# lschoenm/MerKurio

Hardware: AMD Instinct MI355X
Metric: Gbases/s scanned (150bp FASTQ, 10k 31-mers); % HBM roofline at 1/2/4/8 GPUs (higher is better)
Workload: dtype u8

## Files before the change

merkurio_amd/csrc/matcher.cpp:

```cpp
#include <hip/hip_runtime.h>

#include <algorithm>
#include <chrono>
#include <cmath>
#include <cstdarg>
#include <cstdio>
#include <cstdlib>
#include <cstring>
#include <memory>
#include <string>
#include <vector>

#include "host_common.h"
#include "matcher_internal.h"
#include "scan_kernel.h"

namespace mk {

thread_local char g_last_error[512] = "";

int fail(int code, const char *fmt, ...) {
    va_list ap;
    va_start(ap, fmt);
    vsnprintf(g_last_error, sizeof(g_last_error), fmt, ap);
// ... 519 lines not shown
    p.pat_bytes = m->d_pat_bytes;
    p.pat_off = m->d_pat_off;
    p.n_pat = m->n_pat;
    p.q = m->q;
    const uint64_t kmask = m->q >= 32 ? ~0ull : ((1ull << (2 * m->q)) - 1);
    p.key_mask_lo = (uint32_t)kmask;
    p.key_mask_hi = (uint32_t)(kmask >> 32);
    p.case_insensitive = (m->flags & MK_FLAG_ASCII_CASE_INSENSITIVE) ? 1 : 0;
    p.s2 = m->split_len ? m->S2 : 0;
    p.s2_log2 = m->S2 >= 8 ? 3 : m->S2 >= 4 ? 2 : m->S2 >= 2 ? 1 : 0;
    p.key2_mask = (1u << (2 * m->q2)) - 1u;
    p.short_bytes = m->q2 <= kShortByteMaxQ;
    p.short_bitmap = m->d_short_table;
    p.uniform_len = m->uniform_len;
    p.rec_flags32 = (uint32_t *)d_rec_flags;
    p.hits = (mk_hit *)d_hits;
    p.hits_cap = (mode == MK_MODE_HITS) ? hits_cap : 0;
    p.n_hits = (unsigned long long *)d_n_hits;
    p.counters = (unsigned long long *)d_counters;
    p.error_word = m->d_error;
    const uint64_t waves_per_block = kBlockThreads / 64;
    uint64_t blocks = (n_tiles + waves_per_block - 1) / waves_per_block;
    if (blocks > (uint64_t)m->num_cus) blocks = m->num_cus;
    p.stage = m->d_stage;
    p.rec_per_byte = (double)n_rec / (double)n_bytes;
    const uint64_t tiles_per_wave = n_tiles / (blocks * waves_per_block);
    p.tile_run = m->tile_run ? m->tile_run : tiles_per_wave >= 16 ? 4 : tiles_per_wave >= 8 ? 2 : 1;
    p.rec_index = nullptr;
    p.rec_len = rec_len;
    p.inv_rec_len = rec_len ? 1.0 / (double)rec_len : 0.0;
    if (m->ragged && !rec_len && n_rec < (1ull << 32)) {
        int rc_i = ensure((void **)&m->d_rec_index, &m->d_rec_index_cap, ((n_bytes >> kRecIndexShift) + 2) * sizeof(uint32_t));
        if (rc_i) return rc_i;
        launch_rec_index(p.rec_off, n_rec, n_bytes, m->d_rec_index, st);
        p.rec_index = m->d_rec_index;
    }
    const size_t slots = m->ev_start.size();
    const size_t slot = slots ? (size_t)(m->timed_launches % slots) : 0;
    if (slots) MK_HIP(hipEventRecord(m->ev_start[slot], st));
    const uint32_t kDensePerMille = mode == MK_MODE_HITS ? 95 : 145;
    const bool plain_loads = m->hit_density_pm >= kDensePerMille && !m->split_len;
    const int flavour = plain_loads ? 0 : 1;
    const bool listed = !(plain_loads && m->gbloom_blocks == 0) && mode != MK_MODE_HITS && n_rec < (1ull << 32);
    p.flag_list = listed ? m->d_flag_list : nullptr;
    p.flag_counts = m->d_flag_counts;
    p.flag_cap = kFlagListCap;
    const char *name = launch_scan(p, (int)m->S, m->q > 16, mode == MK_MODE_HITS, m->gbloom_blocks != 0, flavour, (int)blocks, st);
    if (!name) return fail(MK_E_UNSUPPORTED, "no kernel for stride %u", m->S);
    if (slots) {
        MK_HIP(hipEventRecord(m->ev_stop[slot], st));
        m->timed_launches++;
    }
    if (listed)
        launch_flag_scatter(m->d_flag_list, m->d_flag_counts, kFlagListCap, (uint32_t)(blocks * waves_per_block), (uint8_t *)d_rec_flags, st);
    if (d_counters) {
        launch_count_flags(p, st);
        if (mode == MK_MODE_HITS && p.hits && p.hits_cap) launch_hist_hits(p, m->num_cus, st);
    }
    m->kernel_name = name;
    m->last_grid = (int)blocks;
    MK_HIP(hipGetLastError());
    return MK_OK;
}

static int take_device_errors(mk_matcher *m, hipStream_t st) {
    uint32_t w = 0;
    MK_HIP(hipMemcpyAsync(&w, m->d_error, sizeof(w), hipMemcpyDeviceToHost, st));
    MK_HIP(hipStreamSynchronize(st));
    if (!w) return MK_OK;
    MK_HIP(hipMemsetAsync(m->d_error, 0, sizeof(w), st));
    return fail(MK_E_UNSUPPORTED, "an occurrence lies 4 GiB or more into its record: a single record must be shorter than 4 GiB "
                                  "(mk_hit.pos is 32 bits); the tuples of that scan are not usable");
}

int mk_matcher_check_device(mk_matcher *m, void *stream) {
    if (!m) return fail(MK_E_INVALID_ARG, "null matcher");
    MK_HIP(hipSetDevice(m->device));
    return take_device_errors(m, (hipStream_t)stream);
}

int mk_matcher_hint_hit_density(mk_matcher *m, uint32_t records_hit_per_1000) {
    if (!m) return fail(MK_E_INVALID_ARG, "null matcher");
    m->hit_density_pm = records_hit_per_1000 > 1000 ? 1000 : records_hit_per_1000;
    return MK_OK;
}

int mk_matcher_set_fixed_record_length(mk_matcher *m, uint32_t record_length) {
    if (!m) return fail(MK_E_INVALID_ARG, "null matcher");
    m->fixed_rec_len = record_length;
    return MK_OK;
}

int mk_matcher_hint_record_lengths(mk_matcher *m, int equal_lengths) {
    if (!m) return fail(MK_E_INVALID_ARG, "null matcher");
    m->ragged = !equal_lengths;
    return MK_OK;
}

int mk_matcher_enable_timing(mk_matcher *m, uint32_t slots) {
    if (!m) return fail(MK_E_INVALID_ARG, "null matcher");
    MK_ABI_BEGIN
    MK_HIP(hipSetDevice(m->device));
    for (auto e : m->ev_start) (void)hipEventDestroy(e);
    for (auto e : m->ev_stop) (void)hipEventDestroy(e);
    m->ev_start.assign(slots, nullptr);
    m->ev_stop.assign(slots, nullptr);
    m->timed_launches = 0;
    for (uint32_t i = 0; i < slots; ++i) {
        MK_HIP(hipEventCreate(&m->ev_start[i]));
// ... 353 lines not shown
```

merkurio_amd/csrc/scan_kernel.h:

```cpp
#pragma once
#include <hip/hip_runtime.h>
#include <stdint.h>

#include "../../include/merkurio_hip.h"
#include "filter.hpp"

namespace mk {

constexpr uint32_t kHitStage = 1024;
constexpr uint32_t kFlagListCap = 2048;

struct ScanParams {
    const uint8_t *seq;
    uint64_t n_bytes;
    const uint64_t *rec_off;
    uint64_t n_rec;
    const uint32_t *bloom;
    uint32_t gbloom_blocks;
    const TableEntry *table;
    uint32_t table_mask;
    const uint8_t *pat_bytes;
    const uint32_t *pat_off;
    uint32_t n_pat;
    uint32_t q;
    uint32_t key_mask_lo;
    uint32_t key_mask_hi;
    uint32_t s2;
    uint32_t s2_log2;
    uint32_t key2_mask;
    uint32_t short_bytes;
    const uint32_t *short_bitmap;
    uint32_t case_insensitive;
    uint32_t uniform_len;
    double rec_per_byte;
    uint32_t tile_run;
    const uint32_t *rec_index;
    uint32_t rec_len;
    double inv_rec_len;
    mk_hit *stage;
    uint32_t *rec_flags32;
    uint32_t *flag_list;
    uint32_t *flag_counts;
    uint32_t flag_cap;
    mk_hit *hits;
    uint64_t hits_cap;
    unsigned long long *n_hits;
    unsigned long long *counters;
    uint32_t *error_word;
};

const char *launch_scan(const ScanParams &p, int S, bool wide, bool emit, bool global_filter, int flavour, int grid_blocks,
                        hipStream_t stream);

template <int S, int QC, bool EMIT, bool GF, int FL, int MC = 0>
void launch_variant(const ScanParams &p, int grid_blocks, hipStream_t stream);

uint32_t scan_lds_bytes();

void launch_hist_hits(const ScanParams &p, int grid_blocks, hipStream_t stream);

constexpr uint32_t kRecIndexShift = 16;
void launch_clear(uint32_t *flags32, uint64_t n_words, unsigned long long *n_hits, hipStream_t stream);
void launch_flag_scatter(const uint32_t *flag_list, const uint32_t *flag_counts, uint32_t flag_cap, uint32_t n_waves, uint8_t *rec_flags,
                         hipStream_t stream);
void launch_rec_index(const uint64_t *rec_off, uint64_t n_rec, uint64_t n_bytes, uint32_t *rec_index, hipStream_t stream);
struct OrderKey {
    const uint32_t *pat_off;
    uint32_t uniform_len;
    const uint32_t *rank;
    const uint32_t *unrank;
    uint64_t rec_base;
    uint32_t ac;
    uint32_t bits_a;
    uint32_t bits_b;
    uint32_t b_hi;
    uint32_t b_lo;
    uint32_t shift;
    uint32_t n_bins;
};
struct OrderScratch {
    unsigned long long *stats;
    uint32_t *g_cnt;
    uint32_t *bin_start;
    uint32_t *cursor;
    uint32_t *big_list;
    uint64_t *keys;
};
constexpr uint32_t kOrderMaxBins = 32768;
constexpr uint32_t kOrderLeafMax = 16384;
constexpr uint32_t kOrderLeafSmall = 4096;
void launch_order_hist(const mk_hit *d_hits, uint64_t n, const OrderKey &L, const OrderScratch &S, int num_cus, hipStream_t st);
void launch_order_scatter_leaf(mk_hit *d_hits, uint64_t n, const OrderKey &L, const OrderScratch &S, uint32_t max_bin, uint32_t n_big,
                               int num_cus, hipStream_t st);
hipError_t order_kernels_prepare();
hipError_t order_hits_library(mk_hit *d_hits, size_t n, bool ac, const uint32_t *d_pat_off, uint32_t uniform_len, void *tmp,
                              size_t *tmp_bytes, hipStream_t stream);

void launch_pattern_sets(const mk_hit *d_hits, uint64_t n, uint64_t n_rec, uint32_t *d_found_pat, unsigned long long *d_found_off,
                         unsigned long long *d_total, void *d_tile, hipStream_t st);
void launch_count_u32(const uint32_t *d_list, uint64_t n, uint32_t *d_counts, uint32_t n_bins, hipStream_t st);
void launch_rows(const mk_hit *d_hits, uint64_t n, uint32_t file, mk_row *d_rows, hipStream_t st);
void launch_pair_mark(mk_hit *d_hits, uint64_t n, uint32_t mate, bool ac, hipStream_t st);
void launch_rows_pair(const mk_hit *d_hits, uint64_t n, bool ac, mk_row *d_rows, hipStream_t st);
void launch_count_pair_heads(const mk_hit *d_hits, uint64_t n, uint32_t *d_counts, uint32_t n_bins, hipStream_t st);

void launch_ingest_count(const uint8_t *d_text, uint64_t n, uint32_t *d_block_cnt, uint32_t *d_total, hipStream_t st);
void launch_ingest_records(const uint8_t *d_text, uint64_t n, const uint32_t *d_block_off, const uint32_t *d_total, uint32_t *d_line_start,
                           uint64_t n_rec, uint32_t *d_rec_start, uint32_t *d_seq_start, uint32_t *d_seq_len, uint32_t *d_status, hipStream_t st);
void launch_ingest_lines(const uint8_t *d_text, uint64_t n, const uint32_t *d_block_off, const uint32_t *d_total, uint32_t *d_line_start, hipStream_t st);
void launch_ingest_offsets(const uint32_t *d_seq_len, uint64_t n_rec, unsigned long long *d_tile, unsigned long long *d_off, hipStream_t st);
void launch_ingest_gather(const uint8_t *d_text, const uint32_t *d_seq_start, const uint32_t *d_seq_len, const unsigned long long *d_off,
                          uint32_t fixed_len, uint64_t n_rec, uint8_t *d_seq, hipStream_t st, uint32_t skip_from = 0xFFFFFFFFu);
void launch_ingest_select(const uint8_t *d_flags, uint32_t invert, const uint32_t *d_rec_start, uint64_t n_rec, uint32_t n_text, uint32_t *d_sel_len,
                          hipStream_t st);
void launch_ingest_fasta_count(const uint8_t *d_text, uint64_t n, const uint32_t *d_nl_block_off, const uint32_t *d_line_start,
                               unsigned long long *d_block64, hipStream_t st);
void launch_ingest_fasta_emit(const uint8_t *d_text, uint64_t n, const uint32_t *d_nl_block_off, const uint32_t *d_line_start,
// ... 71 lines not shown
```

merkurio_amd/csrc/scan_kernel.hip:

```cpp
#include <algorithm>

#include "scan_kernel.h"

namespace mk {

__global__ __launch_bounds__(1024) void mk_count_flags_kernel(const uint8_t *__restrict__ flags, uint64_t n_rec,
                                                             unsigned long long *__restrict__ out) {
    const uint64_t head = std::min<uint64_t>(n_rec, (16 - ((uintptr_t)flags & 15)) & 15);
    const uint64_t n16 = (n_rec - head) / 16;
    const uint4 *__restrict__ v = reinterpret_cast<const uint4 *>(flags + head);
    unsigned long long c = 0;
    const uint64_t stride = (uint64_t)gridDim.x * blockDim.x;
    uint64_t i = (uint64_t)blockIdx.x * blockDim.x + threadIdx.x;
    for (; i + 3 * stride < n16; i += 4 * stride) {
        const uint4 a = v[i], b = v[i + stride], d = v[i + 2 * stride], e = v[i + 3 * stride];
        c += __popc(a.x) + __popc(a.y) + __popc(a.z) + __popc(a.w) + __popc(b.x) + __popc(b.y) + __popc(b.z) + __popc(b.w) +
             __popc(d.x) + __popc(d.y) + __popc(d.z) + __popc(d.w) + __popc(e.x) + __popc(e.y) + __popc(e.z) + __popc(e.w);
    }
    for (; i < n16; i += stride) {
        const uint4 a = v[i];
        c += __popc(a.x) + __popc(a.y) + __popc(a.z) + __popc(a.w);
    }
    if (blockIdx.x == 0 && threadIdx.x == 0) {
        for (uint64_t r = 0; r < head; ++r) c += flags[r] != 0;
        for (uint64_t r = head + n16 * 16; r < n_rec; ++r) c += flags[r] != 0;
    }
    __shared__ unsigned long long part[16];
    for (int o = 32; o > 0; o >>= 1) c += __shfl_down(c, o);
    if ((threadIdx.x & 63) == 0) part[threadIdx.x >> 6] = c;
    __syncthreads();
    if (threadIdx.x == 0) {
        unsigned long long t = 0;
        for (unsigned w = 0; w < blockDim.x / 64; ++w) t += part[w];
        if (t) atomicAdd(out, t);
    }
}

void launch_count_flags(const ScanParams &p, hipStream_t st) {
    const uint64_t n16 = p.n_rec / 16;
    const int blocks = (int)std::min<uint64_t>(256, std::max<uint64_t>(1, (n16 + 4095) / 4096));
    hipLaunchKernelGGL(mk_count_flags_kernel, dim3(blocks), dim3(1024), 0, st, reinterpret_cast<const uint8_t *>(p.rec_flags32),
                       p.n_rec, p.counters + p.n_pat + MK_SUM_RECORDS_HIT);
}

__global__ __launch_bounds__(1024) void mk_clear_kernel(uint32_t *__restrict__ flags32, uint64_t n_words,
                                                       unsigned long long *__restrict__ n_hits) {
    if (blockIdx.x == 0 && threadIdx.x == 0) *n_hits = 0;
    const uint64_t head = std::min<uint64_t>(n_words, ((16 - ((uintptr_t)flags32 & 15)) & 15) / 4);
    const uint64_t n16 = (n_words - head) / 4;
    uint4 *__restrict__ v = reinterpret_cast<uint4 *>(flags32 + head);
    const uint64_t stride = (uint64_t)gridDim.x * blockDim.x;
    for (uint64_t i = (uint64_t)blockIdx.x * blockDim.x + threadIdx.x; i < n16; i += stride) v[i] = make_uint4(0, 0, 0, 0);
    if (blockIdx.x == 0 && threadIdx.x < 8) {
        if (threadIdx.x < head) flags32[threadIdx.x] = 0;
        const uint64_t t = head + n16 * 4 + threadIdx.x;
        if (threadIdx.x < 4 && t < n_words) flags32[t] = 0;
    }
}

void launch_clear(uint32_t *flags32, uint64_t n_words, unsigned long long *n_hits, hipStream_t st) {
    const int blocks = (int)std::min<uint64_t>(512, std::max<uint64_t>(1, (n_words / 4 + 1023) / 1024));
    hipLaunchKernelGGL(mk_clear_kernel, dim3(blocks), dim3(1024), 0, st, flags32, n_words, n_hits);
}

__global__ __launch_bounds__(1024) void mk_flag_scatter_kernel(const uint32_t *__restrict__ list, const uint32_t *__restrict__ counts,
                                                              uint32_t cap, uint32_t n_waves, uint8_t *__restrict__ flags) {
    const uint32_t w = blockIdx.x * (blockDim.x / 64) + threadIdx.x / 64;
    if (w >= n_waves) return;
    const uint32_t n = counts[w] < cap ? counts[w] : cap;
    const uint32_t *__restrict__ l = list + (uint64_t)w * cap;
    for (uint32_t i = threadIdx.x & 63; i < n; i += 64) flags[l[i]] = 1;
}

void launch_flag_scatter(const uint32_t *flag_list, const uint32_t *flag_counts, uint32_t flag_cap, uint32_t n_waves, uint8_t *rec_flags,
                         hipStream_t st) {
    hipLaunchKernelGGL(mk_flag_scatter_kernel, dim3((n_waves + 15) / 16), dim3(1024), 0, st, flag_list, flag_counts, flag_cap, n_waves,
                       rec_flags);
}

constexpr uint32_t kHistLdsBins = 36864;
__global__ __launch_bounds__(1024) void mk_hist_hits_kernel(const mk_hit *__restrict__ hits, const unsigned long long *__restrict__ n_hits,
                                                            uint64_t cap, unsigned long long *__restrict__ counters, uint32_t n_pat) {
    __shared__ uint32_t bins[kHistLdsBins];
    const uint64_t n = std::min<uint64_t>(*n_hits, cap);
    const uint64_t per = std::max<uint64_t>(65536, (n + gridDim.x - 1) / gridDim.x);
    const uint64_t lo = (uint64_t)blockIdx.x * per;
    if (lo >= n) return;
    const uint64_t hi = std::min(n, lo + per);
    const bool in_lds = n_pat <= kHistLdsBins;
    if (in_lds) {
        for (uint32_t i = threadIdx.x; i < n_pat; i += blockDim.x) bins[i] = 0;
        __syncthreads();
    }
    for (uint64_t i = lo + threadIdx.x; i < hi; i += blockDim.x) {
        const uint32_t pat = hits[i].pat;
        if (pat >= n_pat) continue;
        if (in_lds)
            atomicAdd(&bins[pat], 1u);
        else
            atomicAdd(&counters[pat], 1ull);
    }
    if (in_lds) {
        __syncthreads();
        for (uint32_t i = threadIdx.x; i < n_pat; i += blockDim.x)
            if (bins[i]) atomicAdd(&counters[i], (unsigned long long)bins[i]);
    }
}

void launch_hist_hits(const ScanParams &p, int grid_blocks, hipStream_t st) {
    hipLaunchKernelGGL(mk_hist_hits_kernel, dim3(grid_blocks), dim3(1024), 0, st, p.hits, p.n_hits, p.hits_cap, p.counters, p.n_pat);
}

__global__ void mk_rec_index_kernel(const uint64_t *__restrict__ rec_off, uint64_t n_rec, uint64_t n_entries, uint32_t *__restrict__ out) {
    for (uint64_t k = (uint64_t)blockIdx.x * blockDim.x + threadIdx.x; k < n_entries; k += (uint64_t)gridDim.x * blockDim.x) {
        const uint64_t p = k << kRecIndexShift;
        uint64_t lo = 0, hi = n_rec;
        while (hi - lo > 1) {
            const uint64_t mid = (lo + hi) >> 1;
            if (rec_off[mid] <= p)
                lo = mid;
            else
                hi = mid;
        }
        out[k] = (uint32_t)lo;
    }
}

void launch_rec_index(const uint64_t *rec_off, uint64_t n_rec, uint64_t n_bytes, uint32_t *rec_index, hipStream_t stream) {
    const uint64_t n_entries = (n_bytes >> kRecIndexShift) + 2;
    const int blocks = (int)std::min<uint64_t>(2048, (n_entries + 255) / 256);
// ... 203 lines not shown
```

merkurio_amd/csrc/scan_kernel_impl.hpp:

```cpp
#pragma once
#include <algorithm>

#include "scan_kernel.h"

namespace mk {

typedef uint32_t u32x4 __attribute__((ext_vector_type(4)));

__device__ __forceinline__ uint32_t pack4_top(uint32_t d) { return (d & 0x06060606u) * 0x00820820u; }
__device__ __forceinline__ uint32_t pack16(uint4 v) {
    const uint32_t u0 = pack4_top(v.x), u1 = pack4_top(v.y), u2 = pack4_top(v.z), u3 = pack4_top(v.w);
    const uint32_t lo16 = __builtin_amdgcn_perm(u1, u0, 0x0c0c0703u);
    const uint32_t hi16 = __builtin_amdgcn_perm(u3, u2, 0x07030c0cu);
    return lo16 | hi16;
}

__device__ __forceinline__ uint4 load16(const uint8_t *__restrict__ seq, uint64_t pos, uint64_t n) {
    if (pos + 16 <= n) return *reinterpret_cast<const uint4 *>(seq + pos);
    uint32_t w[4] = {0, 0, 0, 0};
    if (pos < n) {
        uint32_t rem = (uint32_t)(n - pos);
        for (uint32_t i = 0; i < rem; ++i) w[i >> 2] |= (uint32_t)seq[pos + i] << (8 * (i & 3));
    }
    return make_uint4(w[0], w[1], w[2], w[3]);
// ... 96 lines not shown
    }
    if (!(rstart <= p && p < rend)) {
        uint64_t hi;
        if (rstart <= p) {
            hi = lo + 1;
            uint64_t step = 1;
            while (hi < n && P.rec_off[hi] <= p) {
                lo = hi;
                step <<= 1;
                hi = (n - hi > step) ? hi + step : n;
            }
        } else {
            hi = lo;
            uint64_t step = 1;
            lo = lo - 1;
            while (P.rec_off[lo] > p) {
                hi = lo;
                step <<= 1;
                lo = lo > step ? lo - step : 0;
            }
        }
        while (hi - lo > 1) {
            const uint64_t mid = (lo + hi) >> 1;
            if (P.rec_off[mid] <= p)
                lo = mid;
            else
                hi = mid;
        }
        rstart = P.rec_off[lo];
        rend = P.rec_off[lo + 1];
    }
    if (p + len > rend) return false;
    if constexpr ((MK_ABLATE & 32) != 0) {
        n_true++;
        return false;
    }
    n_true++;
    out.rec = lo;
    if (EMIT) {
        out.pat = pat;
        out.pos = (uint32_t)(p - rstart);
        if (p - rstart > 0xFFFFFFFFull) atomicOr(P.error_word, 1u);
    }
    return true;
}

struct HitRing {
    uint2 *q;
    uint32_t count;
    mk_hit *stage;
    uint32_t staged;
    uint32_t *flist;
    uint32_t nflag;
};

template <bool FLAGS>
__device__ __forceinline__ void flush_stage(const ScanParams &P, HitRing &hr, uint32_t lane) {
    const uint32_t n = hr.staged;
    if (n == 0) return;
    unsigned long long base = 0;
    if (lane == 0) base = atomicAdd(P.n_hits, (unsigned long long)n);
    const uint32_t blo = __builtin_amdgcn_readfirstlane((uint32_t)base);
    const uint32_t bhi = __builtin_amdgcn_readfirstlane((uint32_t)(base >> 32));
    base = ((unsigned long long)bhi << 32) | blo;
    __builtin_amdgcn_fence(__ATOMIC_RELEASE, "workgroup");
    __builtin_amdgcn_fence(__ATOMIC_ACQUIRE, "workgroup");
    for (uint32_t i = lane; i < n; i += 64) {
        const uint4 v = reinterpret_cast<const uint4 *>(hr.stage)[i];
        if (base + i < P.hits_cap) reinterpret_cast<uint4 *>(P.hits)[base + i] = v;
        if constexpr (FLAGS && (MK_ABLATE & 256) == 0)
            reinterpret_cast<uint8_t *>(P.rec_flags32)[((uint64_t)v.y << 32) | v.x] = 1;
    }
    __builtin_amdgcn_fence(__ATOMIC_RELEASE, "workgroup");
    hr.staged = 0;
}

template <bool EMIT, int FL>
__device__ __forceinline__ void drain_hits(const ScanParams &P, HitRing &hr, uint64_t newest_end, uint32_t lane, uint32_t &n_true) {
    constexpr bool WIDE = FL == 0;
    const uint32_t n = hr.count;
    __builtin_amdgcn_fence(__ATOMIC_RELEASE, "wavefront");
    __builtin_amdgcn_wave_barrier();
    const uint2 e = hr.q[lane & (kHitSlots - 1)];
    __builtin_amdgcn_wave_barrier();
    bool hit = false;
    mk_hit out;
    if (lane < n) {
        uint64_t p = (newest_end & 0xFFFFFFFF00000000ull) | e.x;
        if (p >= newest_end) p -= 1ull << 32;
        hit = resolve_one<EMIT, FL>(P, e.y, p, n_true, out);
    }
    hr.count = 0;
    const uint64_t mm = __ballot(hit);
    if (mm == 0) return;
    const uint32_t below = __builtin_amdgcn_mbcnt_hi((uint32_t)(mm >> 32), __builtin_amdgcn_mbcnt_lo((uint32_t)mm, 0u));
    const uint32_t n_hit = (uint32_t)__popcll(mm);
    if constexpr (EMIT) {
        if constexpr (WIDE && (MK_ABLATE & 256) == 0)
            if (hit) reinterpret_cast<uint8_t *>(P.rec_flags32)[out.rec] = 1;
        if (hit) hr.stage[hr.staged + below] = out;
        hr.staged += n_hit;
        if (hr.staged > kHitStage - 64) flush_stage<!WIDE>(P, hr, lane);
    } else if constexpr ((MK_ABLATE & 256) == 0) {
        if (!WIDE && hr.flist && hr.nflag + n_hit <= P.flag_cap) {
            if (hit) hr.flist[hr.nflag + below] = (uint32_t)out.rec;
            hr.nflag += n_hit;
        } else if (hit) {
            reinterpret_cast<uint8_t *>(P.rec_flags32)[out.rec] = 1;
        }
    }
}

template <bool EMIT, int CS, int FL>
__device__ __forceinline__ bool probe_round(const ScanParams &P, bool active, uint32_t fp, uint32_t ctx, uint64_t t, uint4 v0, uint4 v1,
                                            uint32_t lane, HitRing &hr, uint64_t newest_end, uint32_t &n_true) {
    const uint32_t efp[4] = {v0.x, v0.z, v1.x, v1.z};
    const uint32_t epo[4] = {v0.y, v0.w, v1.y, v1.w};
#pragma unroll
    for (int k = 0; k < 4; ++k) {
        const uint32_t e_off = epo[k] & 15u, e_pat = (epo[k] & ~kBucketOverflow) >> 4;
        uint32_t want = fp;
        if constexpr (CS > 0) want = ctx_fp(fp, ctx & ctx_mask(e_off & (uint32_t)(CS - 1), (uint32_t)CS));
        const bool match = active && epo[k] != kEmptyPat && efp[k] == want && t >= e_off;
        const uint64_t mm = (MK_ABLATE & 64) ? 0ull : __ballot(match);
        if (mm) {
            const uint32_t cnt = (uint32_t)__popcll(mm);
            if (hr.count + cnt > kHitSlots) drain_hits<EMIT, FL>(P, hr, newest_end, lane, n_true);
            if (match) {
                const uint32_t below =
                    __builtin_amdgcn_mbcnt_hi((uint32_t)(mm >> 32), __builtin_amdgcn_mbcnt_lo((uint32_t)mm, 0u));
                hr.q[hr.count + below] = make_uint2((uint32_t)(t - e_off), e_pat);
            }
            hr.count += cnt;
        }
    }
    return active && epo[0] != kEmptyPat && (epo[0] & kBucketOverflow) != 0;
}

__device__ __forceinline__ void load_bucket(const ScanParams &P, bool active, uint32_t b, uint4 &v0, uint4 &v1) {
    v0 = make_uint4(0, kEmptyPat, 0, kEmptyPat);
    v1 = v0;
    if (active) {
        const uint4 *bp = reinterpret_cast<const uint4 *>(P.table + (size_t)b * kBucketEntries);
        v0 = bp[0];
        v1 = bp[1];
    }
}

template <bool EMIT, int CS, int FL>
__device__ __forceinline__ void probe_chain(const ScanParams &P, bool active, uint32_t b, uint32_t fp, uint32_t ctx, uint64_t t,
                                            uint32_t lane, HitRing &hr, uint64_t newest_end, uint32_t &n_true) {
    while (__ballot(active)) {
        uint4 v0, v1;
        load_bucket(P, active, b, v0, v1);
        active = probe_round<EMIT, CS, FL>(P, active, fp, ctx, t, v0, v1, lane, hr, newest_end, n_true);
        b = (b + 1) & P.table_mask;
    }
}

#ifndef MK_ISSUE_AT
#define MK_ISSUE_AT 56
// ... 65 lines not shown
            const uint32_t t = stream32(w0, w1, w2, sh + 24);
            return __umul24(lo, C1) + __umul24(t, C2);
        } else {
            const uint32_t t = stream32(w0, w1, w2, sh + 24);
            constexpr uint32_t top = QC >= 28 ? 0xFF000000u : (((1u << (2 * QC - 48)) - 1u) << 24);
            return __umul24(lo, C1) + __umul24(t, C2) + (t & top);
        }
    } else {
        const uint32_t lo = stream32(w0, w1, w2, sh) & mask_lo;
        const uint32_t hi = QC == 0 ? 0u : (stream32(w0, w1, w2, sh + 32) & mask_hi);
        const uint32_t t = __builtin_amdgcn_alignbit(hi, lo, 24);
        return __umul24(lo, C1) + __umul24(t, C2) + (t & 0xFF000000u);
    }
}

template <int S, int QC, bool EMIT, bool GF, int FL, int MC = 0>
__global__ __launch_bounds__(kBlockThreads) void mk_scan_kernel(const ScanParams P) {
    static_assert(!(MC != 0 && GF && QC > 0), "two length classes with the main filter in global memory: the runtime-q kernels only "
                                              "(the context fingerprints of the fixed-q ones cover the main class's geometry)");
    constexpr bool NTL = FL != 0;
    constexpr bool kCtx = GF && QC > 0;
    constexpr int CS = kCtx ? S : 0;
    using G = Geo<S, QC, kCtx, MC>;
    constexpr bool kPipe = kCtx && G::kNS <= 2 && (MK_ABLATE & 7) == 0;
    constexpr bool kWide = FL == 0;
    constexpr uint32_t kShortWords = MC != 0 ? kShortBitmapWords : 0;
    __shared__ __attribute__((aligned(16))) uint32_t lds_all[kShortWords + kLdsBytes / 4];
    uint32_t *const bloom = lds_all + kShortWords;
    uint32_t *lds_sums = bloom + kBloomWords;
    const uint32_t *short_bm = lds_all;
    if constexpr (!GF) {
        const uint4 *src = reinterpret_cast<const uint4 *>(P.bloom);
        uint4 *dst = reinterpret_cast<uint4 *>(bloom);
        for (uint32_t i = threadIdx.x; i < kBloomWords / 4; i += kBlockThreads) dst[i] = src[i];
    }
    if constexpr (MC != 0) {
        const uint4 *src2 = reinterpret_cast<const uint4 *>(P.short_bitmap);
        uint4 *dst2 = reinterpret_cast<uint4 *>(lds_all);
        for (uint32_t i = threadIdx.x; i < kShortBitmapWords / 4; i += kBlockThreads) dst2[i] = src2[i];
    }
    if constexpr (!GF || MC != 0) __syncthreads();
    const uint2 *__restrict__ gbloom = reinterpret_cast<const uint2 *>(P.bloom);
    const uint32_t gmask = P.gbloom_blocks;

    if (P.counters && blockIdx.x == 0 && threadIdx.x == 0) {
        atomicAdd(&P.counters[P.n_pat + MK_SUM_RECORDS], (unsigned long long)P.n_rec);
        atomicAdd(&P.counters[P.n_pat + MK_SUM_BASES], (unsigned long long)P.n_bytes);
    }
    const uint32_t lane = threadIdx.x & 63u;
    const uint32_t wave_in_block = __builtin_amdgcn_readfirstlane(threadIdx.x >> 6);
    const uint64_t wave_id = (uint64_t)blockIdx.x * (kBlockThreads / 64) + wave_in_block;
    const uint64_t n_waves = (uint64_t)gridDim.x * (kBlockThreads / 64);
    constexpr int NS = G::kNS;
    constexpr uint64_t kTileBytes = (uint64_t)kTileChunks * kChunkBytes;
    const uint32_t mask_lo = P.key_mask_lo, mask_hi = P.key_mask_hi;
    const uint8_t *__restrict__ seq = P.seq;
    const uint64_t n_bytes = P.n_bytes;
    CandEntry *ring = reinterpret_cast<CandEntry *>(bloom + kBloomWords) + wave_in_block * kRingEntries;
    uint32_t *ctx_ring = bloom + wave_in_block * kRingEntries;
    uint32_t q_head = 0, q_count = 0, n_cand = 0;
    HitRing hr;
    hr.q = reinterpret_cast<uint2 *>(bloom + kBloomWords + (kBlockThreads / 64) * kRingEntries * 2) + wave_in_block * kHitSlots;
    hr.count = 0;
    hr.stage = EMIT ? P.stage + wave_id * (uint64_t)kHitStage : nullptr;
    hr.staged = 0;
    hr.flist = (!kWide && !EMIT && P.flag_list) ? P.flag_list + wave_id * (uint64_t)P.flag_cap : nullptr;
    hr.nflag = 0;
    uint32_t n_true = 0;
    uint32_t abl_acc = 0;

    auto halo = [&](uint32_t pk_cur, uint32_t pk_nxt, uint32_t &w1, uint32_t &w2) __attribute__((always_inline)) {
        w1 = 0;
        w2 = 0;
        if constexpr (G::kNeedW1) {
            const uint32_t n0 = __builtin_amdgcn_readlane(pk_nxt, 0);
            w1 = __builtin_amdgcn_update_dpp(n0, pk_cur, 0x130, 0xf, 0xf, false);
        }
        if constexpr (G::kNeedW2) {
            const uint32_t n1 = __builtin_amdgcn_readlane(pk_nxt, 1);
            w2 = __builtin_amdgcn_update_dpp(n1, w1, 0x130, 0xf, 0xf, false);
        }
    };
    auto filter_chunk = [&](uint32_t pk_cur, uint32_t pk_nxt, uint32_t &h0, uint32_t &h1) __attribute__((always_inline)) -> uint32_t {
        const uint32_t w0 = pk_cur;
        uint32_t w1, w2;
        halo(pk_cur, pk_nxt, w1, w2);
        if constexpr ((MK_ABLATE & 4) != 0) return ((w0 ^ w1 ^ w2) == 0x12345678u) ? 1u : 0u;
        uint32_t cand = 0;
        const char *bloom_bytes = reinterpret_cast<const char *>(bloom);
#pragma unroll
        for (int j = 0; j < NS; ++j) {
            uint32_t h = sample_hash<S, QC>(w0, w1, w2, 2 * j * S, mask_lo, mask_hi);
            if (j == 0) h0 = h;
            if (j == 1) h1 = h;
            uint2 blk;
            if constexpr ((MK_ABLATE & 2) != 0) {
                blk = make_uint2(h & 0x10101010u, h);
            } else if constexpr (GF) {
                blk = gbloom[gbloom_block(h, gmask)];
                h = gbloom_bits(h);
            } else {
                blk = *reinterpret_cast<const uint2 *>(bloom_bytes + bloom_block_byte(h));
            }
            uint32_t m = (blk.x >> (h >> 27)) & (blk.y >> (h >> 22)) & (blk.y >> (h >> 17));
            if constexpr (GF) m &= blk.x >> (h >> 12);
            cand |= (m & 1u) << j;
        }
        if constexpr (MC != 0) {
            uint32_t c2;
#if defined(MK_MC_ABL) && MK_MC_ABL == 1
            c2 = 0;
#elif defined(MK_MC_ABL) && MK_MC_ABL == 2
            c2 = short_filter<4, true>(short_bm, w0, w1, P.key2_mask);
#else
            if constexpr (MC > 1) {
                c2 = short_filter<MC, true>(short_bm, w0, w1, P.key2_mask);
            } else if (P.short_bytes) {
                switch (P.s2) {
                    case 1: c2 = short_filter<1, true>(short_bm, w0, w1, P.key2_mask); break;
                    case 2: c2 = short_filter<2, true>(short_bm, w0, w1, P.key2_mask); break;
// ... 67 lines not shown
        if (q_count > 64) drain_ring(64);
        if (slot_full) {
            const uint32_t below =
                __builtin_amdgcn_mbcnt_hi((uint32_t)(full >> 32), __builtin_amdgcn_mbcnt_lo((uint32_t)full, 0u));
            CandEntry e;
            e.h = slot_h;
            e.t_lo = slot_t;
            ring[(q_head + q_count + below) & (kRingEntries - 1)] = e;
            if constexpr (kCtx) ctx_ring[(q_head + q_count + below) & (kRingEntries - 1)] = slot_c;
        }
        q_count += (uint32_t)__popcll(full);
        n_cand += (uint32_t)__popcll(full);
        slot_full = false;
    };
    auto queue_candidates = [&](uint32_t pk_cur, uint32_t pk_nxt, uint32_t wm1, uint32_t cand, uint64_t cpos, uint32_t h0, uint32_t h1) __attribute__((always_inline)) {
        const uint32_t w0 = pk_cur;
        uint32_t w1 = 0, w2 = 0;
        if constexpr (NS > 2 || kCtx || MC != 0) halo(pk_cur, pk_nxt, w1, w2);
        newest_end = cpos + kChunkBytes;
        const uint32_t t_base = (uint32_t)cpos + lane * 16;
        do {
            if (__ballot(cand != 0 && slot_full)) flush_slots();
            if (cand != 0) {
                const uint32_t j = (uint32_t)__ffs(cand) - 1u;
                cand &= cand - 1;
                if constexpr (NS <= 2) {
                    slot_h = j ? h1 : h0;
                } else {
                    const uint32_t sh = 2u * j * S;
                    const uint32_t klo = __builtin_amdgcn_alignbit(w1, w0, sh) & mask_lo;
                    const uint32_t khi = __builtin_amdgcn_alignbit(w2, w1, sh) & mask_hi;
                    const uint32_t t = __builtin_amdgcn_alignbit(khi, klo, 24);
                    slot_h = __umul24(klo, 0x9E3779u) + __umul24(t, 0x85EBCBu) + (t & 0xFF000000u);
                }
                if constexpr (kCtx) {
                    const uint32_t pb = 2u * j * S;
                    const uint32_t prev7 = pb >= 14u ? (w0 >> (pb - 14u)) : __builtin_amdgcn_alignbit(w0, wm1, (pb + 18u) & 31u);
                    const uint32_t next7 = stream32_rt(w0, w1, w2, pb + 2u * (uint32_t)QC);
                    slot_c = (prev7 & 0x3FFFu) | ((next7 & 0x3FFFu) << 14);
                }
                slot_t = t_base + j * S;
                if constexpr (MC != 0) {
                    const uint32_t j2 = (j - 16u) << P.s2_log2;
                    const uint32_t fp2 = short_fp(__builtin_amdgcn_alignbit(w1, w0, 2u * j2) & P.key2_mask);
                    const bool is2 = j >= 16u;
                    slot_h = is2 ? fp2 : main_fp(slot_h);
                    slot_t = is2 ? t_base + j2 : slot_t;
                }
                slot_full = true;
            }
        } while (__ballot(cand != 0));
    };

    const uint64_t n_main_tiles = n_bytes >= kChunkBytes ? (n_bytes - kChunkBytes) / kTileBytes : 0;
    if (wave_id * (P.tile_run ? P.tile_run : 1u) < n_main_tiles) {
        const uint32_t run = P.tile_run ? P.tile_run : 1u;
        const uint64_t jump = (n_waves - 1) * (uint64_t)run + 1;
        uint64_t ld_tile = wave_id * run;
        uint32_t ld_run = 0;
        uint32_t ld_g = 0;
        const uint64_t last_tile = n_main_tiles - 1;
        const uint8_t *ld_ptr = seq + (ld_tile < last_tile ? ld_tile : last_tile) * kTileBytes + lane * 16;
        auto nt_load = [](const uint8_t *p) -> uint4 {
            if constexpr (NTL) {
                const u32x4 nv = __builtin_nontemporal_load(reinterpret_cast<const u32x4 *>(p));
                return make_uint4(nv.x, nv.y, nv.z, nv.w);
            } else {
                return *reinterpret_cast<const uint4 *>(p);
            }
        };
        auto load_group = [&](uint4 &a, uint4 &b, uint4 &c, uint4 &d) __attribute__((always_inline)) {
            a = nt_load(ld_ptr);
            b = nt_load(ld_ptr + kChunkBytes);
            c = nt_load(ld_ptr + 2 * kChunkBytes);
            d = nt_load(ld_ptr + 3 * kChunkBytes);
            ld_ptr += 4 * kChunkBytes;
            if (++ld_g == (uint32_t)(kTileChunks + 1) / 4) {
                ld_g = 0;
                if (++ld_run == run) {
                    ld_run = 0;
                    ld_tile += jump;
                } else {
                    ld_tile += 1;
                }
                const uint64_t t = ld_tile < last_tile ? ld_tile : last_tile;
                ld_ptr = seq + t * kTileBytes + lane * 16;
            }
        };
        uint4 r0, r1, r2, r3;
        load_group(r0, r1, r2, r3);
        uint32_t pk_prev = 0;
        uint32_t pk_pp = 0, pk_tile_prev = 0;
        bool pd_on = false;
        uint32_t pd_h0 = 0, pd_h1 = 0, pd_cur = 0, pd_nxt = 0, pd_wm1 = 0;
        uint2 pd_b0 = make_uint2(0, 0), pd_b1 = pd_b0;
        uint64_t pd_cpos = 0;
        auto test_pending = [&]() __attribute__((always_inline)) {
            auto pass = [](uint32_t h, uint2 blk) -> uint32_t {
                const uint32_t hb = gbloom_bits(h);
                return (blk.x >> (hb >> 27)) & (blk.x >> (hb >> 12)) & (blk.y >> (hb >> 22)) & (blk.y >> (hb >> 17)) & 1u;
            };
            uint32_t cand = pass(pd_h0, pd_b0);
            if constexpr (NS > 1) cand |= pass(pd_h1, pd_b1) << 1;
            if (__ballot(cand != 0)) queue_candidates(pd_cur, pd_nxt, pd_wm1, cand, pd_cpos, pd_h0, pd_h1);
        };
        uint64_t last_push_base = 0;
        uint32_t sc_run = 0;
        for (uint64_t tile = wave_id * run; tile < n_main_tiles;) {
            const uint64_t base = tile * kTileBytes;
            if constexpr (kCtx) {
                pk_tile_prev = 0;
                if (base >= 16) pk_tile_prev = pack16(*reinterpret_cast<const uint4 *>(seq + base - 16));
            }
            if (base - last_push_base >= (1ull << 30)) {
                last_push_base = base;
                flush_slots();
                if (hr.count) drain_hits<EMIT, FL>(P, hr, newest_end, lane, n_true);
                if (q_count && !pend_on) issue_probe(q_count < 64 ? q_count : 64);
            }
#pragma unroll 1
            for (int g = 0; g < (kTileChunks + 1) / 4; ++g) {
                const uint32_t p0 = pack16(r0), p1 = pack16(r1), p2 = pack16(r2), p3 = pack16(r3);
                asm volatile("" ::"v"(p0), "v"(p1), "v"(p2), "v"(p3) : "memory");
                if (pend_on) consume_probe();
                load_group(r0, r1, r2, r3);
                {
                    uint32_t q0 = p0, q1 = p1, q2 = p2;
#pragma unroll 1
                    for (int k = 0; k < 4; ++k) {
                        const int ci = 4 * g + k - 1;
                        if constexpr (kPipe) {
                            uint32_t nh0 = 0, nh1 = 0, nwm1 = 0;
                            uint2 nb0 = make_uint2(0, 0), nb1 = nb0;
                            if (ci >= 0) {
                                uint32_t w1, w2;
                                halo(pk_prev, q0, w1, w2);
                                nh0 = sample_hash<S, QC>(pk_prev, w1, w2, 0, mask_lo, mask_hi);
                                nb0 = gbloom[gbloom_block(nh0, gmask)];
                                if constexpr (NS > 1) {
                                    nh1 = sample_hash<S, QC>(pk_prev, w1, w2, 2 * S, mask_lo, mask_hi);
                                    nb1 = gbloom[gbloom_block(nh1, gmask)];
                                }
                                nwm1 = __builtin_amdgcn_update_dpp(__builtin_amdgcn_readlane(pk_pp, 63), pk_prev, 0x138, 0xf, 0xf, false);
                            }
                            if (pd_on) test_pending();
                            pd_on = ci >= 0;
                            pd_h0 = nh0;
                            pd_h1 = nh1;
                            pd_b0 = nb0;
                            pd_b1 = nb1;
                            pd_cur = pk_prev;
                            pd_nxt = q0;
                            pd_wm1 = nwm1;
                            pd_cpos = base + (uint64_t)(ci < 0 ? 0 : ci) * kChunkBytes;
                        } else if (ci >= 0) {
                            uint32_t h0 = 0, h1 = 0;
                            const uint32_t ck = filter_chunk(pk_prev, q0, h0, h1);
                            if constexpr ((MK_ABLATE & 4) != 0) n_cand += ck;
                            if (__ballot(ck != 0)) {
                                uint32_t wm1 = 0;
                                if constexpr (kCtx)
                                    wm1 = __builtin_amdgcn_update_dpp(__builtin_amdgcn_readlane(pk_pp, 63), pk_prev, 0x138, 0xf, 0xf, false);
                                queue_candidates(pk_prev, q0, wm1, ck, base + (uint64_t)ci * kChunkBytes, h0, h1);
                            }
                        }
                        if constexpr (kCtx) pk_pp = ci < 0 ? pk_tile_prev : pk_prev;
                        pk_prev = q0;
                        q0 = q1;
                        q1 = q2;
                        q2 = p3;
                    }
                }
                if constexpr ((MK_ABLATE & 8) != 0) {
                    if (q_count >= MK_ISSUE_AT) {
                        q_head = (q_head + q_count) & (kRingEntries - 1);
                        q_count = 0;
                    }
                } else if (!pend_on && q_count >= (FL == 0 ? MK_ISSUE_AT_DENSE : MK_ISSUE_AT)) {
                    issue_probe(q_count < 64 ? q_count : 64);
                }
                if constexpr (FL == 0 && MK_DRAIN_AT_DENSE <= 64) {
                    if (hr.count >= MK_DRAIN_AT_DENSE) drain_hits<EMIT, FL>(P, hr, newest_end, lane, n_true);
                }
                pk_prev = p3;
            }
            if (++sc_run == run) {
                sc_run = 0;
                tile += jump;
            } else {
                tile += 1;
            }
        }
        if constexpr (kPipe) {
            if (pd_on) test_pending();
        }
    }
    if (pend_on) consume_probe();

    {
        const uint64_t tail_rank = (wave_id + n_waves - (n_main_tiles / (P.tile_run ? P.tile_run : 1u)) % n_waves) % n_waves;
        for (uint64_t cpos = n_main_tiles * kTileBytes + tail_rank * kChunkBytes; cpos < n_bytes; cpos += n_waves * kChunkBytes) {
            const uint32_t pk_cur = pack16(load16(seq, cpos + lane * 16, n_bytes));
            const uint32_t pk_nxt = pack16(load16(seq, cpos + kChunkBytes + lane * 16, n_bytes));
            uint32_t h0 = 0, h1 = 0;
            const uint32_t ck = filter_chunk(pk_cur, pk_nxt, h0, h1);
            if constexpr ((MK_ABLATE & 4) != 0) n_cand += ck;
            if (__ballot(ck != 0)) {
                uint32_t wm1 = 0;
                if constexpr (kCtx) {
                    const uint64_t mine = cpos + lane * 16;
                    if (mine >= 16) wm1 = pack16(load16(seq, mine - 16, n_bytes));
                }
                queue_candidates(pk_cur, pk_nxt, wm1, ck, cpos, h0, h1);
            }
        }
    }

    flush_slots();
    while (q_count) drain_ring(q_count < 64 ? q_count : 64);
    if (hr.count) drain_hits<EMIT, FL>(P, hr, newest_end, lane, n_true);
    if constexpr (EMIT) flush_stage<!kWide>(P, hr, lane);
    if (hr.flist && lane == 0) P.flag_counts[wave_id] = hr.nflag;
    if ((MK_ABLATE & 1) != 0 && abl_acc == 0xFFFFFFFFu) n_cand++;
    if (P.counters) {
        __syncthreads();
        if (threadIdx.x < kLdsSumWords) lds_sums[threadIdx.x] = 0;
        __syncthreads();
        if (lane == 0 && n_cand) atomicAdd(&lds_sums[0], n_cand);
        if (n_true) atomicAdd(&lds_sums[1], n_true);
        __syncthreads();
        if (threadIdx.x == 0 && lds_sums[0]) atomicAdd(&P.counters[P.n_pat + MK_SUM_CANDIDATES], (unsigned long long)lds_sums[0]);
        if (threadIdx.x == 1 && lds_sums[1]) atomicAdd(&P.counters[P.n_pat + MK_SUM_HITS], (unsigned long long)lds_sums[1]);
    }
}

}
```

Baseline: 6195.

## Count newly hit records during flag setting and merge tile runs into contiguous spans

Record flags are now set with a byte-lane atomicOr on 32-bit words, and each set that flips a flag is counted. The records-hit counter is therefore accumulated inside the scan and scatter kernels, and the separate count-flags pass over the whole flag array is skipped when the flag list path is used. Separately, the main scan loop replaces its tile/run/jump bookkeeping with contiguous spans of tile_run tiles strided by wave count, which simplifies the load and scan indexing. The cost is an atomic per flagged record in place of a plain byte store, and span length now covers overlapping group boundaries differently, which could change tail coverage.

```diff
diff --git a/merkurio_amd/csrc/matcher.cpp b/merkurio_amd/csrc/matcher.cpp
--- a/merkurio_amd/csrc/matcher.cpp
+++ b/merkurio_amd/csrc/matcher.cpp
@@ -595,9 +595,10 @@
         m->timed_launches++;
     }
     if (listed)
-        launch_flag_scatter(m->d_flag_list, m->d_flag_counts, kFlagListCap, (uint32_t)(blocks * waves_per_block), (uint8_t *)d_rec_flags, st);
+        launch_flag_scatter(m->d_flag_list, m->d_flag_counts, kFlagListCap, (uint32_t)(blocks * waves_per_block), (uint32_t *)d_rec_flags,
+                            d_counters ? p.counters + p.n_pat + MK_SUM_RECORDS_HIT : nullptr, st);
     if (d_counters) {
-        launch_count_flags(p, st);
+        if (!listed) launch_count_flags(p, st);
         if (mode == MK_MODE_HITS && p.hits && p.hits_cap) launch_hist_hits(p, m->num_cus, st);
     }
     m->kernel_name = name;
diff --git a/merkurio_amd/csrc/scan_kernel.h b/merkurio_amd/csrc/scan_kernel.h
--- a/merkurio_amd/csrc/scan_kernel.h
+++ b/merkurio_amd/csrc/scan_kernel.h
@@ -61,8 +61,8 @@
 
 constexpr uint32_t kRecIndexShift = 16;
 void launch_clear(uint32_t *flags32, uint64_t n_words, unsigned long long *n_hits, hipStream_t stream);
-void launch_flag_scatter(const uint32_t *flag_list, const uint32_t *flag_counts, uint32_t flag_cap, uint32_t n_waves, uint8_t *rec_flags,
-                         hipStream_t stream);
+void launch_flag_scatter(const uint32_t *flag_list, const uint32_t *flag_counts, uint32_t flag_cap, uint32_t n_waves, uint32_t *rec_flags32,
+                         unsigned long long *records_hit, hipStream_t stream);
 void launch_rec_index(const uint64_t *rec_off, uint64_t n_rec, uint64_t n_bytes, uint32_t *rec_index, hipStream_t stream);
 struct OrderKey {
     const uint32_t *pat_off;
diff --git a/merkurio_amd/csrc/scan_kernel.hip b/merkurio_amd/csrc/scan_kernel.hip
--- a/merkurio_amd/csrc/scan_kernel.hip
+++ b/merkurio_amd/csrc/scan_kernel.hip
@@ -64,18 +64,35 @@
 }
 
 __global__ __launch_bounds__(1024) void mk_flag_scatter_kernel(const uint32_t *__restrict__ list, const uint32_t *__restrict__ counts,
-                                                              uint32_t cap, uint32_t n_waves, uint8_t *__restrict__ flags) {
+                                                              uint32_t cap, uint32_t n_waves, uint32_t *__restrict__ flags32,
+                                                              unsigned long long *__restrict__ records_hit) {
     const uint32_t w = blockIdx.x * (blockDim.x / 64) + threadIdx.x / 64;
-    if (w >= n_waves) return;
-    const uint32_t n = counts[w] < cap ? counts[w] : cap;
-    const uint32_t *__restrict__ l = list + (uint64_t)w * cap;
-    for (uint32_t i = threadIdx.x & 63; i < n; i += 64) flags[l[i]] = 1;
-}
-
-void launch_flag_scatter(const uint32_t *flag_list, const uint32_t *flag_counts, uint32_t flag_cap, uint32_t n_waves, uint8_t *rec_flags,
-                         hipStream_t st) {
+    uint32_t c = 0;
+    if (w < n_waves) {
+        const uint32_t n = counts[w] < cap ? counts[w] : cap;
+        const uint32_t *__restrict__ l = list + (uint64_t)w * cap;
+        for (uint32_t i = threadIdx.x & 63; i < n; i += 64) {
+            const uint32_t rec = l[i];
+            const uint32_t bit = 1u << (8u * (rec & 3u));
+            c += (atomicOr(flags32 + (rec >> 2), bit) & bit) ? 0u : 1u;
+        }
+    }
+    if (!records_hit) return;
+    __shared__ uint32_t part[16];
+    for (int o = 32; o > 0; o >>= 1) c += __shfl_down(c, o);
+    if ((threadIdx.x & 63) == 0) part[threadIdx.x >> 6] = c;
+    __syncthreads();
+    if (threadIdx.x == 0) {
+        unsigned long long t = 0;
+        for (unsigned k = 0; k < blockDim.x / 64; ++k) t += part[k];
+        if (t) atomicAdd(records_hit, t);
+    }
+}
+
+void launch_flag_scatter(const uint32_t *flag_list, const uint32_t *flag_counts, uint32_t flag_cap, uint32_t n_waves, uint32_t *rec_flags32,
+                         unsigned long long *records_hit, hipStream_t st) {
     hipLaunchKernelGGL(mk_flag_scatter_kernel, dim3((n_waves + 15) / 16), dim3(1024), 0, st, flag_list, flag_counts, flag_cap, n_waves,
-                       rec_flags);
+                       rec_flags32, records_hit);
 }
 
 constexpr uint32_t kHistLdsBins = 36864;
diff --git a/merkurio_amd/csrc/scan_kernel_impl.hpp b/merkurio_amd/csrc/scan_kernel_impl.hpp
--- a/merkurio_amd/csrc/scan_kernel_impl.hpp
+++ b/merkurio_amd/csrc/scan_kernel_impl.hpp
@@ -172,7 +172,13 @@
     uint32_t staged;
     uint32_t *flist;
     uint32_t nflag;
+    uint32_t n_newflag;
 };
+
+__device__ __forceinline__ uint32_t set_flag_counted(uint32_t *__restrict__ flags32, uint64_t rec) {
+    const uint32_t bit = 1u << (8u * ((uint32_t)rec & 3u));
+    return (atomicOr(flags32 + (rec >> 2), bit) & bit) ? 0u : 1u;
+}
 
 template <bool FLAGS>
 __device__ __forceinline__ void flush_stage(const ScanParams &P, HitRing &hr, uint32_t lane) {
@@ -226,7 +232,10 @@
             if (hit) hr.flist[hr.nflag + below] = (uint32_t)out.rec;
             hr.nflag += n_hit;
         } else if (hit) {
-            reinterpret_cast<uint8_t *>(P.rec_flags32)[out.rec] = 1;
+            if (!WIDE && hr.flist)
+                hr.n_newflag += set_flag_counted(P.rec_flags32, out.rec);
+            else
+                reinterpret_cast<uint8_t *>(P.rec_flags32)[out.rec] = 1;
         }
     }
 }
@@ -398,7 +407,6 @@
     const uint64_t wave_id = (uint64_t)blockIdx.x * (kBlockThreads / 64) + wave_in_block;
     const uint64_t n_waves = (uint64_t)gridDim.x * (kBlockThreads / 64);
     constexpr int NS = G::kNS;
-    constexpr uint64_t kTileBytes = (uint64_t)kTileChunks * kChunkBytes;
     const uint32_t mask_lo = P.key_mask_lo, mask_hi = P.key_mask_hi;
     const uint8_t *__restrict__ seq = P.seq;
     const uint64_t n_bytes = P.n_bytes;
@@ -412,6 +420,7 @@
     hr.staged = 0;
     hr.flist = (!kWide && !EMIT && P.flag_list) ? P.flag_list + wave_id * (uint64_t)P.flag_cap : nullptr;
     hr.nflag = 0;
+    hr.n_newflag = 0;
     uint32_t n_true = 0;
     uint32_t abl_acc = 0;
 
@@ -585,15 +594,14 @@
         } while (__ballot(cand != 0));
     };
 
-    const uint64_t n_main_tiles = n_bytes >= kChunkBytes ? (n_bytes - kChunkBytes) / kTileBytes : 0;
-    if (wave_id * (P.tile_run ? P.tile_run : 1u) < n_main_tiles) {
-        const uint32_t run = P.tile_run ? P.tile_run : 1u;
-        const uint64_t jump = (n_waves - 1) * (uint64_t)run + 1;
-        uint64_t ld_tile = wave_id * run;
-        uint32_t ld_run = 0;
+    const uint32_t span_groups = (P.tile_run ? P.tile_run : 1u) * (uint32_t)((kTileChunks + 1) / 4);
+    const uint64_t span_bytes = (uint64_t)(span_groups * 4u - 1u) * kChunkBytes;
+    const uint64_t n_spans = n_bytes >= kChunkBytes ? (n_bytes - kChunkBytes) / span_bytes : 0;
+    if (wave_id < n_spans) {
+        uint64_t ld_span = wave_id;
         uint32_t ld_g = 0;
-        const uint64_t last_tile = n_main_tiles - 1;
-        const uint8_t *ld_ptr = seq + (ld_tile < last_tile ? ld_tile : last_tile) * kTileBytes + lane * 16;
+        const uint64_t last_span = n_spans - 1;
+        const uint8_t *ld_ptr = seq + ld_span * span_bytes + lane * 16;
         auto nt_load = [](const uint8_t *p) -> uint4 {
             if constexpr (NTL) {
                 const u32x4 nv = __builtin_nontemporal_load(reinterpret_cast<const u32x4 *>(p));
@@ -608,16 +616,11 @@
             c = nt_load(ld_ptr + 2 * kChunkBytes);
             d = nt_load(ld_ptr + 3 * kChunkBytes);
             ld_ptr += 4 * kChunkBytes;
-            if (++ld_g == (uint32_t)(kTileChunks + 1) / 4) {
+            if (++ld_g == span_groups) {
                 ld_g = 0;
-                if (++ld_run == run) {
-                    ld_run = 0;
-                    ld_tile += jump;
-                } else {
-                    ld_tile += 1;
-                }
-                const uint64_t t = ld_tile < last_tile ? ld_tile : last_tile;
-                ld_ptr = seq + t * kTileBytes + lane * 16;
+                ld_span += n_waves;
+                const uint64_t t = ld_span < last_span ? ld_span : last_span;
+                ld_ptr = seq + t * span_bytes + lane * 16;
             }
         };
         uint4 r0, r1, r2, r3;
@@ -638,9 +641,8 @@
             if (__ballot(cand != 0)) queue_candidates(pd_cur, pd_nxt, pd_wm1, cand, pd_cpos, pd_h0, pd_h1);
         };
         uint64_t last_push_base = 0;
-        uint32_t sc_run = 0;
-        for (uint64_t tile = wave_id * run; tile < n_main_tiles;) {
-            const uint64_t base = tile * kTileBytes;
+        for (uint64_t span = wave_id; span < n_spans; span += n_waves) {
+            const uint64_t base = span * span_bytes;
             if constexpr (kCtx) {
                 pk_tile_prev = 0;
                 if (base >= 16) pk_tile_prev = pack16(*reinterpret_cast<const uint4 *>(seq + base - 16));
@@ -652,7 +654,7 @@
                 if (q_count && !pend_on) issue_probe(q_count < 64 ? q_count : 64);
             }
 #pragma unroll 1
-            for (int g = 0; g < (kTileChunks + 1) / 4; ++g) {
+            for (int g = 0; g < (int)span_groups; ++g) {
                 const uint32_t p0 = pack16(r0), p1 = pack16(r1), p2 = pack16(r2), p3 = pack16(r3);
                 asm volatile("" ::"v"(p0), "v"(p1), "v"(p2), "v"(p3) : "memory");
                 if (pend_on) consume_probe();
@@ -717,12 +719,6 @@
                 }
                 pk_prev = p3;
             }
-            if (++sc_run == run) {
-                sc_run = 0;
-                tile += jump;
-            } else {
-                tile += 1;
-            }
         }
         if constexpr (kPipe) {
             if (pd_on) test_pending();
@@ -731,8 +727,8 @@
     if (pend_on) consume_probe();
 
     {
-        const uint64_t tail_rank = (wave_id + n_waves - (n_main_tiles / (P.tile_run ? P.tile_run : 1u)) % n_waves) % n_waves;
-        for (uint64_t cpos = n_main_tiles * kTileBytes + tail_rank * kChunkBytes; cpos < n_bytes; cpos += n_waves * kChunkBytes) {
+        const uint64_t tail_rank = (wave_id + n_waves - n_spans % n_waves) % n_waves;
+        for (uint64_t cpos = n_spans * span_bytes + tail_rank * kChunkBytes; cpos < n_bytes; cpos += n_waves * kChunkBytes) {
             const uint32_t pk_cur = pack16(load16(seq, cpos + lane * 16, n_bytes));
             const uint32_t pk_nxt = pack16(load16(seq, cpos + kChunkBytes + lane * 16, n_bytes));
             uint32_t h0 = 0, h1 = 0;
@@ -761,7 +757,9 @@
         __syncthreads();
         if (lane == 0 && n_cand) atomicAdd(&lds_sums[0], n_cand);
         if (n_true) atomicAdd(&lds_sums[1], n_true);
+        if (hr.n_newflag) atomicAdd(&lds_sums[2], hr.n_newflag);
         __syncthreads();
+        if (threadIdx.x == 2 && lds_sums[2]) atomicAdd(&P.counters[P.n_pat + MK_SUM_RECORDS_HIT], (unsigned long long)lds_sums[2]);
         if (threadIdx.x == 0 && lds_sums[0]) atomicAdd(&P.counters[P.n_pat + MK_SUM_CANDIDATES], (unsigned long long)lds_sums[0]);
         if (threadIdx.x == 1 && lds_sums[1]) atomicAdd(&P.counters[P.n_pat + MK_SUM_HITS], (unsigned long long)lds_sums[1]);
     }
```

After: 6112. 1.3% lower.
